# ai3DVision/CP_PFDR_graph_d1

Measured on AMD Instinct MI355X. Metric: PFDR iter/s and Medge-updates/s, 10M-vertex 6-NN graph, 1/2/4/8 MI355X, higher is better.
Workload: dtype f32; 1 GPU; PFDR_graph_quadratic_d1_l1<float>, identity A, l1 + TV, jittered 250x200x200 grid, 6-NN (V=10000000, E=60000000); global_graph=250x200x200, V_per_gpu=10000000, E_per_gpu=60000000, parallelism=single, device_inputs=True, device_bytes=3010452620, relabelled=False, split_incidence_blocks=0, tiled_blocks=39063, record_blocks=39063, slot_patterns=0, sequential_evolution=False, speculation=none, finite=True

## Files before the change

### cp_pfdr_graph_d1_amd/csrc/pfdr_quadratic.hip

```cpp
#include <cstring>
#include <stdexcept>

#include "pfdr_loop.hpp"
#include "pfdr_order.hpp"
#include "pfdr_quadratic_kernels.hpp"
#include "pfdr_sort.hpp"
#include "pfdr_sparse.hpp"
#include "pfdr_sparse_view.hpp"

namespace pfdr {

template <typename T>
static void permute(DevBuf<T> &d, const int *map, size_t n, hipStream_t s) {
    if (!d.p || !n) return;
    DevBuf<T> t(n);
    k_gather<T><<<grid_for(n), kBlock, 0, s>>>((long)n, d.p, map, t.p);
    PFDR_HIP(hipGetLastError());
    std::swap(d.p, t.p);
    std::swap(d.n, t.n);
}

__global__ void k_edge_order_keys(long E, const int *__restrict__ Eu, const int *__restrict__ where,
                                  unsigned long long *__restrict__ keys, unsigned *__restrict__ vals) {
    const long e = (long)blockIdx.x * blockDim.x + threadIdx.x;
// ... 1328 lines not shown
}

template <typename real>
void QuadSession<real>::edge_sweep(long ebeg, long eend, const Ctrl<real> *c, const char *name,
                                   long ebeg2, long eend2, const FuseDecide<real> *fd) {
    constexpr int EPT = Vec<real>::kPer16B;
    if (eend <= ebeg) { ebeg = ebeg2; eend = eend2; ebeg2 = eend2 = 0; }
    if (eend <= ebeg) return;
    hipStream_t s = stream;
    ProfScope ps(prof, name, s);
    ERange rg{ebeg, eend, ebeg2, eend2, grid_for(eend - ebeg, EPT)};
    const int nb = rg.nb0 + (eend2 > ebeg2 ? grid_for(eend2 - ebeg2, EPT) : 0);
    const int xm = xcd_fit(nb, xcd_e_), g = xcd_grid(nb, xm);
    const FuseDecide<real> f = fd ? *fd : FuseDecide<real>{};
    if (ends_ && fuse_) {
        k_edge_sweep_ends<real><<<g, kBlock, 0, s>>>(E_, xpe_.p, gie_.p, Z2_.p, A1_.p, cw_,
                                                     la_it(), la0_, rho_, c, nb, xm, f, pad_out());
        return;
    }
    constexpr long EB = kBlock * EPT;
    if (tiled_ && !fuse_ && rg.nb0 == nb && ebeg % EB == 0 && (eend % EB == 0 || eend == E_)) {
        auto k = rr_.p ? k_edge_sweep_tl<real, true, true>
                 : (!la_it() && !A1_.p) ? k_edge_sweep_tl<real, true>
                                        : k_edge_sweep_tl<real, false>;
        k<<<g, kBlock, 0, s>>>(E_, V_, Eu_.p, luv_.p, erec_.p, Ev_.p, xr_, Z2_.p, A1_.p, cw_,
                               gi_.p, la_it(), la0_, zdirect() ? nullptr : wz_.p, rho_, c,
                               (int)(ebeg / EB), nb, xm, rr_.p);
        return;
    }
    if (tiled_) throw std::logic_error("tiled edge sweep: range not on edge blocks");
    if (us_ && uptr_.p) {
        auto k = fuse_ ? k_edge_sweep_us<real, true> : k_edge_sweep_us<real, false>;
        k<<<g, kBlock, 0, s>>>(E_, Eu_.p, Ev_.p, uptr_.p, xr_, Z2_.p, A1_.p, cw_, gi_.p,
                               la_it(), la0_, wz_.p, rho_, c, nb, xm, rg, f, pad_out());
    } else {
        auto k = fuse_ ? k_edge_sweep<real, true> : k_edge_sweep<real, false>;
        k<<<g, kBlock, 0, s>>>(E_, Eu_.p, Ev_.p, xr_, Z2_.p, A1_.p, cw_, gi_.p, la_it(), la0_,
                               wz_.p, rho_, c, nb, xm, rg, f, pad_out());
    }
}

template <typename real>
void QuadSession<real>::tiny_chunk(int n) {
    const bool gated = track_ || rec_obj_;
    TinyArgs<real> t{};
    t.E = E_; t.Eu = Eu_.p; t.Ev = Ev_.p; t.Z2 = Z2_.p; t.A1 = A1_.p; t.La_d1 = la_it();
    t.la0 = la0_; t.cw = cw_; t.rho = rho_; t.gi = gi_.p; t.wz = wz_.p;
    t.va = vargs(0, nbv_, nullptr);
    t.red = red_.p; t.ctrl = gated ? ctrl_.p : nullptr; t.Dif = rec_dif_ ? Dif_.p : nullptr;
    t.track = track_ ? 1 : 0; t.iters = n;
    ProfScope ps(prof, "tiny_iterate", stream);
    k_tiny_iterate<real><<<1, kTiny, 0, stream>>>(t);
    PFDR_HIP(hipGetLastError());
}

template <typename real>
VArgs<real> QuadSession<real>::vargs(int bbeg, int bend, const Ctrl<real> *c) {
    VArgs<real> a{};
    a.V = V_; a.ptr = inc_.ptr.p; a.idx = inc_.idx.p; a.xp = xr_; a.wz = wz_.p;
    a.xpo = xw_ == xr_ ? nullptr : xw_;
    a.uptr = uptr_.p; a.mask = mask_.p; a.oidx = oidx_.p; a.blkok = blkok_.p;
    a.Y = Y_.p; a.A = A_.p; a.Ga = Ga_.p; a.Th_l1 = Th_l1_.p;
    a.prox = prox_; a.positivity = positivity_; a.lo = lo_; a.hi = hi_;
    a.fwd = mode_ == A_IDENT ? 1 : (mode_ == A_DIAG ? 2 : 0);
    a.track = track_ ? 1 : 0; a.part = vpart_.p; a.ctrl = c;
    a.late = fuse_ ? 1 : 0;
    a.E = E_;
    if (tiled_) {
        a.slots = slots_.p; a.trec = trec_.p; a.ptab = ptab_.p; a.prec = prec_.p; a.deg8 = deg8_.p; a.ustart = ustart_.p; a.tptr = tptr_.p; a.tstart = tstart_.p;
        a.tlen = tlen_.p; a.tok = tok_.p;
        a.zs = Z2_.p; a.invAux = invAux_.p; a.a0 = cw_ * la0_;
        a.gi = gi_.p;
    }
    a.l1uni = l1_uniform_ ? 1 : 0;
    a.l1u = l1u_;
    a.terms = seqdif_ ? terms_.p : nullptr;
    a.tmap = seqdif_ && reordered_ ? order_.p : nullptr;
    a.tstride = tstride_;
    a.bbeg = bbeg; a.nb = bend - bbeg; a.xcd = xcd_fit(a.nb, xcd_v_);
    a.bsplit = a.nb; a.bjump = 0;
    return a;
}

template <typename real>
void QuadSession<real>::vertex_sweep(int bbeg, int bend, const Ctrl<real> *c, const char *name,
                                     int bbeg2, int bend2) {
    if (bend <= bbeg) { bbeg = bbeg2; bend = bend2; bbeg2 = bend2 = 0; }
    if (bend <= bbeg) return;
    hipStream_t s = stream;
    VArgs<real> a = vargs(bbeg, bend, c);
    if (bend2 > bbeg2) {
        a.bsplit = bend - bbeg;
        a.bjump = bbeg2 - bend;
        a.nb += bend2 - bbeg2;
        a.xcd = xcd_fit(a.nb, xcd_v_);
    }
    ProfScope ps(prof, name, s);
    if (pad_ && bend2 <= bbeg2) {
        k_vertex_sweep_pad<real><<<xcd_grid(a.nb, a.xcd), kBlock, 0, s>>>(
            a, wzp_.p, pad_nmax_, ends_ ? pidx_.p : nullptr, ends_ ? xpe_.p : nullptr);
        return;
    }
    if (vpair_cap_ && bend2 <= bbeg2 && a.nb >= 2) {
        const int np = a.nb / 2;
        const size_t lb = 2 * (size_t)vpair_cap_ * sizeof(real);
        if (a.nb & 1) {
            VArgs<real> a1 = a;
            a1.bbeg = a.bbeg + a.nb - 1;
            a1.nb = 1;
            a1.bsplit = 1;
            a1.xcd = 0;
            if (zdirect()) k_vertex_sweep<real, 8, true><<<1, kBlock, 0, s>>>(a1);
            else k_vertex_sweep<real, 8><<<1, kBlock, 0, s>>>(a1);
        }
        a.xcd = xcd_fit(np, xcd_v_);
        const int g = xcd_grid(np, a.xcd);
        if (zdirect()) k_vertex_sweep_pair<real, true><<<g, kBlock, lb, s>>>(a, vpair_cap_);
        else k_vertex_sweep_pair<real><<<g, kBlock, lb, s>>>(a, vpair_cap_);
        return;
    }
    if (zdirect())
        k_vertex_sweep<real, 8, true><<<xcd_grid(a.nb, a.xcd), kBlock, 0, s>>>(a);
    else
        k_vertex_sweep<real, 8><<<xcd_grid(a.nb, a.xcd), kBlock, 0, s>>>(a);
}

template <typename real>
void QuadSession<real>::sweeps(const Ctrl<real> *c) {
    hipStream_t s = stream;
    if (overlap_) {
        PFDR_HIP(hipEventRecord(ev_[0], s));
        PFDR_HIP(hipStreamWaitEvent(comm_, ev_[0], 0));
        {
            ProfScope ps(prof, "halo_pull", comm_);
            halo_->pull(xr_, sizeof(R2<real>), comm_);
        }
        PFDR_HIP(hipEventRecord(ev_[1], comm_));
        edge_sweep(elo_, ehi_, c, "edge_sweep");
        PFDR_HIP(hipStreamWaitEvent(s, ev_[1], 0));
        edge_sweep(0, elo_, c, "edge_sweep_b", ehi_, E_);
        PFDR_HIP(hipEventRecord(ev_[2], s));
        PFDR_HIP(hipStreamWaitEvent(comm_, ev_[2], 0));
        {
            ProfScope ps(prof, "halo_push", comm_);
            real *src = zdirect() ? Z2_.p : wz_.p;
            halo_->push(src, src + 2 * E_, sizeof(real), comm_);
        }
        PFDR_HIP(hipEventRecord(ev_[3], comm_));
        vertex_sweep(blo_, bhi_, c, "vertex_sweep");
        PFDR_HIP(hipStreamWaitEvent(s, ev_[3], 0));
        vertex_sweep(0, blo_, c, "vertex_sweep_b", bhi_, nbv_);
    } else {
        if (halo_) {
            ProfScope ps(prof, "halo_pull", s);
            halo_->pull(xr_, sizeof(R2<real>), s);
        }
        edge_sweep(0, E_, c, "edge_sweep");
        if (halo_) {
            ProfScope ps(prof, "halo_push", s);
            real *src = zdirect() ? Z2_.p : wz_.p;
            halo_->push(src, src + 2 * E_, sizeof(real), s);
        }
        vertex_sweep(0, nbv_, c, "vertex_sweep");
    }
}

template <typename real>
void QuadSession<real>::spec_sweeps(int t, int b) {
    xr_ = xpb(t - 1);
    xw_ = xpb(t);
    real *const keep = terms_.p, *const keepp = vpart_.p;
    terms_.p += (long)b * 2 * tstride_;
    vpart_.p += (long)b * 2 * nbv_;
    sweeps(ctrl_.p);
    terms_.p = keep;
    vpart_.p = keepp;
    xr_ = xw_ = xp_.p;
}

template <typename real>
void QuadSession<real>::spec_decide(int b, hipStream_t s) {
    seq_evolution(terms_.p + (long)b * 2 * tstride_, vpart_.p + (long)b * 2 * nbv_, s);
    k_decide<real><<<1, 64, 0, s>>>(ctrl_.p, red_.p, rec_dif_ ? Dif_.p : nullptr, 1);
}

template <typename real>
void QuadSession<real>::body(int i, int n) {
    hipStream_t s = stream;
    const bool gated = track_ || rec_obj_;
    const Ctrl<real> *c = gated ? ctrl_.p : nullptr;
    if (fuse_) {
        Ctrl<real> *cb[2] = {ctrl_.p, ctrl2_.p};
        FuseDecide<real> fd{};
        if (i > 0) {
            fd.src = cb[(i - 1) & 1]; fd.dst = cb[i & 1]; fd.part = vpart_.p;
            fd.red = red_.p; fd.Dif = rec_dif_ ? Dif_.p : nullptr; fd.nparts = nbv_;
        }
        edge_sweep(0, E_, cb[0], "edge_sweep", 0, 0, &fd);
        vertex_sweep(0, nbv_, cb[i & 1], "vertex_sweep");
        if (i == n - 1) {
            FuseDecide<real> fl{cb[i & 1], cb[0], vpart_.p, red_.p, rec_dif_ ? Dif_.p : nullptr,
                                nbv_};
            k_decide_fused<real><<<1, kBlock, 0, s>>>(fl);
        }
        PFDR_HIP(hipGetLastError());
        return;
    }
// ... 308 lines not shown
```

### cp_pfdr_graph_d1_amd/csrc/pfdr_quadratic_kernels.hpp

```cpp
#pragma once
#include <algorithm>
#include <cmath>
#include <cstring>
#include <memory>
#include <type_traits>

#include "pfdr_graph.hpp"
#include "pfdr_monosum.hpp"
#include "pfdr_session.hpp"

namespace pfdr {

enum AMode : int { A_IDENT = 0, A_DIAG = 1, A_DIRECT = 2, A_ATA = 3 };
enum Prox : int { PROX_NONE = 0, PROX_L1 = 1, PROX_POS = 2, PROX_BOX = 3,
                  PROX_LO = 4, PROX_HI = 5 };
enum Gate : int { GATE_NONE = 0, GATE_ACTIVE = 1, GATE_OBJ = 2,
                  GATE_ACTIVE_OR_OBJ = 3 };

template <typename real> using R2 = typename Vec<real>::v2;

template <typename T, int N>
__device__ __forceinline__ Pk<T, N> ldv(const T *p) {
    return *reinterpret_cast<const Pk<T, N> *>(p);
}
// ... 183 lines not shown
            acc += __shfl(ng, kWave - 1, kWave);
        }
    }
    {
        const long fu = us / G;
        const int ngu = nu > 0 ? (int)((us + nu - 1) / G - fu + 1) : 0;
        for (int b = 0; b < ngu; b += kBlock * GG) {
            Slots12 d[GG];
            Pk<real, VE> x[GG][ZV];
#pragma unroll
            for (int u = 0; u < GG; u++) {
                const long g = fu + min(b + u * kBlock + tid, ngu - 1);
                d[u] = slots[g];
#pragma unroll
                for (int z = 0; z < ZV; z++) x[u][z] = ldv<real, VE>(wz + g * G + z * VE);
            }
#pragma unroll
            for (int u = 0; u < GG; u++) {
                const int k = b + u * kBlock + tid;
                if (k < ngu) {
                    const long base = (fu + k) * G;
#pragma unroll
                    for (int q = 0; q < G; q++)
                        if (base + q >= us && base + q < (long)us + nu)
                            lds[slot12(d[u], q)] = x[u][q / VE].v[q % VE];
                }
            }
        }
    }
    __syncthreads();
    const int ngv = nt ? rp[nt - 1] : 0;
    int lo = 0, end = nt ? rp[0] : 0, beg = 0;
    for (int b = 0; b < ngv; b += kBlock * GG) {
        Slots12 d[GG];
        Pk<real, VE> x[GG][ZV];
        long base[GG], A[GG];
        int L[GG];
#pragma unroll
        for (int u = 0; u < GG; u++) {
            const int k = min(b + u * kBlock + tid, ngv - 1);
            while (end <= k) {
                beg = end;
                end = rp[++lo];
            }
            A[u] = E + rs[lo];
            L[u] = rl[lo];
            base[u] = (A[u] / G + (k - beg)) * G;
        }
#pragma unroll
        for (int u = 0; u < GG; u++) {
            d[u] = slots[base[u] / G];
#pragma unroll
            for (int z = 0; z < ZV; z++) x[u][z] = ldv<real, VE>(wz + base[u] + z * VE);
        }
#pragma unroll
        for (int u = 0; u < GG; u++)
            if (b + u * kBlock + tid < ngv) {
#pragma unroll
                for (int q = 0; q < G; q++)
                    if (base[u] + q >= A[u] && base[u] + q < A[u] + L[u])
                        lds[slot12(d[u], q)] = x[u][q / VE].v[q % VE];
            }
    }
    __syncthreads();
    int my0 = dinc - dg;
    for (int q = 0; q < w; q++) my0 += wt[q];
    const int my1 = my0 + dg;
    real s = real(0);
    int j = my0;
    for (; j + 4 <= my1; j += 4) {
        const real a0 = lds[j], a1 = lds[j + 1], a2 = lds[j + 2], a3 = lds[j + 3];
        s += ZD ? wv * a0 : a0;
        s += ZD ? wv * a1 : a1;
        s += ZD ? wv * a2 : a2;
        s += ZD ? wv * a3 : a3;
    }
    for (; j < my1; j++) s += ZD ? wv * lds[j] : lds[j];
    return s;
}

constexpr int kRecRuns = 14, kTileRec = 32;
constexpr int kPrec = 16;

template <typename real, bool ZD = false>
__device__ __forceinline__ real tile_sum_rec(int V, long E, int blk, int v,
                                             const unsigned char *__restrict__ deg8,
                                             const Slots12 *__restrict__ slots,
                                             const int *__restrict__ trec,
                                             const real *__restrict__ wz, real *lds, int *wt,
                                             real wv = real(1),
                                             const Slots12 *__restrict__ ptab = nullptr,
                                             const int *__restrict__ prec = nullptr,
                                             bool pre = false, int pre_rv = 0, int pre_pr = 0,
                                             int pre_dg = 0) {
    constexpr int VE = Vec<real>::kPer16B, G = kSlotGroup, ZV = G / VE;
    const int tid = threadIdx.x, lane = tid & (kWave - 1), w = tid / kWave;
    const int dg = pre ? pre_dg : v < V ? deg8[v] : 0;
    const int rv = pre ? pre_rv : lane < kTileRec ? trec[(long)blk * kTileRec + lane] : 0;
    const int pr = pre ? pre_pr : prec && lane < kPrec ? prec[(long)blk * kPrec + lane] : 0;
    int dinc = dg;
#pragma unroll
    for (int o = 1; o < kWave; o <<= 1) {
        const int y = __shfl_up(dinc, o, kWave);
        if (lane >= o) dinc += y;
    }
    if (lane == kWave - 1) wt[w] = dinc;
    const int us = __builtin_amdgcn_readlane(rv, 0), nu = __builtin_amdgcn_readlane(rv, 1);
    const int nt = __builtin_amdgcn_readlane(rv, 2);
    const int st = __shfl(rv, min(3 + 2 * lane, kWave - 1), kWave);
    const int ln = __shfl(rv, min(4 + 2 * lane, kWave - 1), kWave);
    int P = 0;
    if (lane < nt && ln > 0) {
        const long A = E + st;
        P = (int)((A + ln - 1) / G - A / G + 1);
    }
#pragma unroll
    for (int o = 1; o < kWave; o <<= 1) {
        const int y = __shfl_up(P, o, kWave);
        if (lane >= o) P += y;
    }
    const int ngv = __builtin_amdgcn_readlane(P, kWave - 1);
    const long fu = us / G;
    const int ngu = nu > 0 ? (int)((us + nu - 1) / G - fu + 1) : 0;
    const int tot = ngu + ngv;
    for (int b = 0; b < tot; b += 2 * kBlock) {
        Slots12 d[2];
        Pk<real, VE> x[2][ZV];
        long gb[2], lo[2], hi[2];
        int pg[2];
#pragma unroll
        for (int u = 0; u < 2; u++) {
            const int k = min(b + u * kBlock + tid, tot - 1);
            const int kv = k - ngu;
            int r = 0;
            for (int q = 0; q < nt; q++) r += __builtin_amdgcn_readlane(P, q) <= kv;
            r = min(r, kWave - 1);
            const int sr = __shfl(st, r, kWave), lr = __shfl(ln, r, kWave);
            const int pb = __shfl(P, max(r - 1, 0), kWave);
            const int pv = __shfl(pr, min(r + 1, kWave - 1), kWave);
            if (k < ngu) {
                gb[u] = fu + k;
                lo[u] = us;
                hi[u] = (long)us + nu;
                pg[u] = __builtin_amdgcn_readlane(pr, 0) + k;
            } else {
                const long A = E + sr;
                const int gi = kv - (r > 0 ? pb : 0);
                gb[u] = A / G + gi;
                lo[u] = A;
                hi[u] = A + lr;
                pg[u] = pv + gi;
            }
        }
#pragma unroll
        for (int u = 0; u < 2; u++) {
            d[u] = prec ? ptab[pg[u]] : slots[gb[u]];
#pragma unroll
            for (int z = 0; z < ZV; z++) x[u][z] = ldv<real, VE>(wz + gb[u] * G + z * VE);
        }
#pragma unroll
        for (int u = 0; u < 2; u++)
            if (b + u * kBlock + tid < tot) {
#pragma unroll
                for (int q = 0; q < G; q++) {
                    const long p = gb[u] * G + q;
                    if (p >= lo[u] && p < hi[u]) lds[slot12(d[u], q)] = x[u][q / VE].v[q % VE];
                }
            }
    }
    __syncthreads();
    int my0 = dinc - dg;
    for (int q = 0; q < w; q++) my0 += wt[q];
    const int my1 = my0 + dg;
    real s = real(0);
    int j = my0;
    for (; j + 4 <= my1; j += 4) {
        const real a0 = lds[j], a1 = lds[j + 1], a2 = lds[j + 2], a3 = lds[j + 3];
        s += ZD ? wv * a0 : a0;
        s += ZD ? wv * a1 : a1;
        s += ZD ? wv * a2 : a2;
        s += ZD ? wv * a3 : a3;
    }
    for (; j < my1; j++) s += ZD ? wv * lds[j] : lds[j];
    return s;
}

template <typename real, bool ZD = false>
__device__ __forceinline__ void tile_sum_rec2(int V, long E, int b0, int v0, int v1,
                                              const unsigned char *__restrict__ deg8,
                                              const Slots12 *__restrict__ slots,
                                              const int *__restrict__ trec,
                                              const real *__restrict__ wz, real *lds, int cap,
                                              int *wt, real wv0, real wv1,
                                              const Slots12 *__restrict__ ptab,
                                              const int *__restrict__ prec, real &x0, real &x1) {
    static_assert(kTileRec == 32 && kWave == 64 && kPrec == 16, "two records per wave register");
    constexpr int VE = Vec<real>::kPer16B, G = kSlotGroup, ZV = G / VE, NW = kBlock / kWave;
    const int tid = threadIdx.x, lane = tid & (kWave - 1), w = tid / kWave;
    const int dg0 = v0 < V ? deg8[v0] : 0, dg1 = v1 < V ? deg8[v1] : 0;
    const int rv = trec[(long)b0 * kTileRec + lane];
    const int pr = prec ? prec[(long)b0 * kPrec + (lane & 31)] : 0;
    int i0 = dg0, i1 = dg1;
#pragma unroll
    for (int o = 1; o < kWave; o <<= 1) {
        const int y0 = __shfl_up(i0, o, kWave), y1 = __shfl_up(i1, o, kWave);
        if (lane >= o) {
            i0 += y0;
            i1 += y1;
        }
    }
    if (lane == kWave - 1) {
        wt[w] = i0;
        wt[NW + w] = i1;
    }
    const int us0 = __builtin_amdgcn_readlane(rv, 0), nu0 = __builtin_amdgcn_readlane(rv, 1);
    const int nt0 = __builtin_amdgcn_readlane(rv, 2);
    const int us1 = __builtin_amdgcn_readlane(rv, 32), nu1 = __builtin_amdgcn_readlane(rv, 33);
    const int nt1 = __builtin_amdgcn_readlane(rv, 34);
    const int hf = lane >> 5, rl = lane & 31;
    const int st = __shfl(rv, 32 * hf + min(3 + 2 * rl, 31), kWave);
    const int ln = __shfl(rv, 32 * hf + min(4 + 2 * rl, 31), kWave);
    int P = 0;
    if (rl < (hf ? nt1 : nt0) && ln > 0) {
        const long A = E + st;
        P = (int)((A + ln - 1) / G - A / G + 1);
    }
#pragma unroll
    for (int o = 1; o < 32; o <<= 1) {
        const int y = __shfl_up(P, o, kWave);
        if (rl >= o) P += y;
    }
    const int ngv0 = __builtin_amdgcn_readlane(P, 31), ngv1 = __builtin_amdgcn_readlane(P, 63);
    const long fu0 = us0 / G, fu1 = us1 / G;
    const int ngu0 = nu0 > 0 ? (int)((us0 + nu0 - 1) / G - fu0 + 1) : 0;
    const int ngu1 = nu1 > 0 ? (int)((us1 + nu1 - 1) / G - fu1 + 1) : 0;
    const int tot0 = ngu0 + ngv0, tot = tot0 + ngu1 + ngv1;
    const int pu0 = __builtin_amdgcn_readlane(pr, 0), pu1 = __builtin_amdgcn_readlane(pr, 16);
    for (int b = 0; b < tot; b += 2 * kBlock) {
        Slots12 d[2];
        Pk<real, VE> x[2][ZV];
        long gb[2];
        int pg[2], mt[2];
#pragma unroll
        for (int u = 0; u < 2; u++) {
            const int k = min(b + u * kBlock + tid, tot - 1);
            const int h = k >= tot0;
            const int kk = k - (h ? tot0 : 0);
            const int ngu = h ? ngu1 : ngu0;
            const int kv = kk - ngu;
            int ra = 0, rb = 0;
            for (int q = 0; q < nt0; q++) ra += __builtin_amdgcn_readlane(P, q) <= kv;
            for (int q = 0; q < nt1; q++) rb += __builtin_amdgcn_readlane(P, 32 + q) <= kv;
            const int r = min(h ? rb : ra, 31), base = 32 * h;
            const int sr = __shfl(st, base + r, kWave), lr = __shfl(ln, base + r, kWave);
            const int pb = __shfl(P, base + max(r - 1, 0), kWave);
            const int pv = __shfl(pr, 16 * h + min(r + 1, 15), kWave);
            long L, H;
            if (kk < ngu) {
                gb[u] = (h ? fu1 : fu0) + kk;
                L = h ? us1 : us0;
                H = L + (h ? nu1 : nu0);
                pg[u] = (h ? pu1 : pu0) + kk;
            } else {
                const long A = E + sr;
                const int gi = kv - (r > 0 ? pb : 0);
                gb[u] = A / G + gi;
                L = A;
                H = A + lr;
                pg[u] = pv + gi;
            }
            const int lo = (int)max(L - gb[u] * G, -1L), hi = (int)min(H - gb[u] * G, (long)G + 1);
            mt[u] = (lo + 1) | (hi + 1) << 4 | h << 8;
        }
#pragma unroll
        for (int u = 0; u < 2; u++) {
            d[u] = prec ? ptab[pg[u]] : slots[gb[u]];
#pragma unroll
            for (int z = 0; z < ZV; z++) x[u][z] = ldv<real, VE>(wz + gb[u] * G + z * VE);
        }
#pragma unroll
        for (int u = 0; u < 2; u++)
            if (b + u * kBlock + tid < tot) {
                real *l = lds + ((mt[u] >> 8) ? cap : 0);
                const int lo = (mt[u] & 15) - 1, hi = ((mt[u] >> 4) & 15) - 1;
#pragma unroll
                for (int q = 0; q < G; q++)
                    if (q >= lo && q < hi) l[slot12(d[u], q)] = x[u][q / VE].v[q % VE];
            }
    }
    __syncthreads();
    int my0 = i0 - dg0, my1 = i1 - dg1;
    for (int q = 0; q < w; q++) {
        my0 += wt[q];
        my1 += wt[NW + q];
    }
    real s0 = real(0), s1 = real(0);
    for (int j = 0; j < dg0; j++) s0 += ZD ? wv0 * lds[my0 + j] : lds[my0 + j];
    for (int j = 0; j < dg1; j++) s1 += ZD ? wv1 * lds[cap + my1 + j] : lds[cap + my1 + j];
    x0 = s0;
    x1 = s1;
}

static __global__ void k_tile_keys(long E, const int *__restrict__ Eu, const int *__restrict__ Ev,
                                   int vbits, unsigned long long *__restrict__ keys,
                                   unsigned *__restrict__ vals, int V = 0, bool split = false) {
    const long e = (long)blockIdx.x * blockDim.x + threadIdx.x;
    if (e >= E) return;
    const int u = Eu[e], v = Ev[e];
    const unsigned long long g = split && (u >= V || v >= V) ? 1ull << (2 * vbits) : 0ull;
    keys[e] = g | ((unsigned long long)(u / kBlock) << vbits) | (unsigned)(v / kBlock);
    vals[e] = (unsigned)e;
}

static __global__ void k_count_below(long n, const unsigned long long *__restrict__ keys,
                                     unsigned long long bound, unsigned long long *out) {
    long lo = 0, hi = n;
    while (lo < hi) {
        const long mid = (lo + hi) >> 1;
        if (keys[mid] < bound) lo = mid + 1;
        else hi = mid;
    }
    *out = (unsigned long long)lo;
}

static __global__ void k_tile_slots(int V, const int *__restrict__ ptr,
                                    const unsigned *__restrict__ idx,
                                    unsigned short *__restrict__ d2) {
    const int v = blockIdx.x * blockDim.x + threadIdx.x;
    if (v >= V) return;
    const int base = ptr[v - v % kBlock];
    for (int j = ptr[v]; j < ptr[v + 1]; j++) d2[idx[j]] = (unsigned short)(j - base);
}

static __global__ void k_pack_slots(long ngroups, long n, const unsigned short *__restrict__ d2,
                                    Slots12 *__restrict__ out) {
    const long g = (long)blockIdx.x * blockDim.x + threadIdx.x;
    if (g >= ngroups) return;
    unsigned long long lo = 0, hi = 0;
#pragma unroll
    for (int q = 0; q < kSlotGroup; q++) {
        const long p = g * kSlotGroup + q;
        const unsigned long long x = p < n ? (d2[p] & 0xfffu) : 0u;
        const int bit = 12 * q;
        if (bit + 12 <= 64) {
            lo |= x << bit;
        } else if (bit >= 64) {
            hi |= x << (bit - 64);
        } else {
            lo |= x << bit;
            hi |= x >> (64 - bit);
        }
    }
    Slots12 r;
    r.w[0] = (unsigned)lo;
    r.w[1] = (unsigned)(lo >> 32);
    r.w[2] = (unsigned)hi;
    out[g] = r;
}

static __global__ void k_tile_ustart(long E, int nb, const int *__restrict__ Eu,
                                     int *__restrict__ ustart) {
    const long p = (long)blockIdx.x * blockDim.x + threadIdx.x;
    if (p > E) return;
    const int lo = p == 0 ? 0 : Eu[p - 1] / kBlock + 1;
    const int hi = p == E ? nb : Eu[p] / kBlock;
    for (int b = lo; b <= hi; b++) ustart[b] = (int)p;
}

__device__ __forceinline__ int run_block(long i, const int *__restrict__ a,
                                         const unsigned long long *__restrict__ keys, int V) {
    const int x = keys ? (int)(keys[i] >> 32) : a[i];
    return x < V ? x / kBlock : -1;
}
// ... 1362 lines not shown
#pragma unroll
            for (int j = 0; j < EPT; j++) a.v[j] = cw * la.v[j];
        }
        Pk<real, EPT> ou, ov;
#pragma unroll
        for (int j = 0; j < EPT; j++)
            edge_full<real>(pu[j], pv[j], gu[j], gv[j], a.v[j], la.v[j], z.v[2 * j],
                            z.v[2 * j + 1], ou.v[j], ov.v[j], rho);
        stv<real, 2 * EPT>(Z2 + 2 * e0, z);
        if (pd.sl) {
#pragma unroll
            for (int j = 0; j < EPT; j++) {
                pd.wzp[sv.v[2 * j]] = ou.v[j];
                pd.wzp[sv.v[2 * j + 1]] = ov.v[j];
            }
        } else {
            stv<real, EPT>(wz + e0, ou);
            stv<real, EPT>(wz + E + e0, ov);
        }
    } else {
        for (long e = e0; e < eend; e++) {
            const int u = Eu[e], v = Ev[e];
            real zu = Z2[2 * e], zv = Z2[2 * e + 1], ou, ov;
            const real l = la_at(e, La_d1, la0);
            edge_full<real>(xp[u], xp[v], gi[u], gi[v], A1 ? A1[e] : cw * l, l, zu, zv, ou, ov,
                            rho);
            Z2[2 * e] = zu;
            Z2[2 * e + 1] = zv;
            if (pd.sl) {
                pd.wzp[pd.sl[2 * e]] = ou;
                pd.wzp[pd.sl[2 * e + 1]] = ov;
            } else {
                wz[e] = ou;
                wz[E + e] = ov;
            }
        }
    }
}

template <typename real>
struct VArgs {
    int V;
    int nb, xcd;
    int bbeg;
    int bsplit, bjump;
    const int *ptr;
    const unsigned *idx;
    const int *uptr;
    const unsigned *mask, *oidx;
    const int *blkok;
    const real *wz;
    R2<real> *xp;
    R2<real> *xpo;
    const real *Y, *A, *Ga, *Th_l1;
    int prox, positivity;
    real lo, hi;
    int fwd;
    int track;
    real *part;
    const Ctrl<real> *ctrl;
    int late;
    long E;
    const Slots12 *slots;
    const int *trec;
    const Slots12 *ptab;
    const int *prec;
    const unsigned char *deg8;
    const int *ustart, *tptr, *tstart, *tlen, *tok;
    const real *zs;
    const real *invAux;
    real a0;
    const R2<real> *gi;
    int l1uni;
    real l1u;
    real *terms;
    const int *tmap;
    long tstride;
};

template <typename real> struct VSweep;
template <> struct VSweep<float> { static constexpr int waves = 8; };
template <> struct VSweep<double> { static constexpr int waves = 4; };

template <typename real>
struct VOps {
    R2<real> q{};
    real th = real(0), yv = real(0), gv = real(0), av = real(0), ia = real(0);
};
template <typename real>
__device__ __forceinline__ VOps<real> vertex_ops(const VArgs<real> &a, int v,
                                                 const R2<real> *gpre = nullptr) {
    VOps<real> o;
    if (v < a.V) {
        if (a.track || !a.fwd) o.q = a.xp[v];
        real g = real(0);
        if (a.gi) {
            const R2<real> p = gpre ? *gpre : a.gi[v];
            g = p.x;
            o.ia = p.y;
        } else if (a.fwd || a.l1uni) {
            g = a.Ga[v];
        }
        if (a.prox == PROX_L1) o.th = a.l1uni ? g * a.l1u : a.Th_l1[v];
        if (a.fwd) { o.yv = a.Y[v]; o.gv = g; }
        if (a.fwd == 2) o.av = a.A[v];
    }
    return o;
}

template <typename real>
__device__ __forceinline__ R2<real> vertex_finish(const VArgs<real> &a, int v, real x,
                                                  const VOps<real> &o, real &num, real &den) {
    num = real(0);
    den = real(0);
    R2<real> q = o.q;
    const real th = o.th, yv = o.yv, gv = o.gv, av = o.av;
    if (v < a.V) {
        switch (a.prox) {
            case PROX_L1: {
                if (x > th) x -= th;
                else if (!a.positivity && (x < -th)) x += th;
                else x = real(0);
            } break;
            case PROX_POS:
                if (x < real(0)) x = real(0);
                break;
            case PROX_BOX:
                if (x < a.lo) x = a.lo;
                else if (x > a.hi) x = a.hi;
                break;
            case PROX_LO:
                if (x < a.lo) x = a.lo;
                break;
            case PROX_HI:
                if (x > a.hi) x = a.hi;
                break;
            default:
                break;
        }
        if (a.track) {
            const real d = q.x - x;
            num = d * d;
            den = x * x;
            if (a.terms) {
                const long i = a.tmap ? a.tmap[v] : v;
                a.terms[i] = num;
                a.terms[a.tstride + i] = den;
            }
        }
        q.x = x;
        if (a.fwd) {
            real p = (a.fwd == 2) ? av * x : x;
            p -= yv;
            q.y = real(2) * x - gv * p;
        }
        (a.xpo ? a.xpo : a.xp)[v] = q;
    }
    return q;
}

template <typename real, int GB, bool ZD = false>
__device__ __forceinline__ void vertex_block(const VArgs<real> &a, int blk, real *lds,
                                             real (*red)[kBlock / kWave], int *scan,
                                             int halt = 0) {
    const int v0 = blk * kBlock;
    const int v = v0 + threadIdx.x;
    const VOps<real> o = vertex_ops(a, v);
    const real wv = ZD && v < a.V ? a.a0 * (a.gi ? o.ia : a.invAux[v]) : real(1);
    real x;
    const bool pre = a.slots && a.trec;
    int pre_rv = 0, pre_pr = 0, pre_dg = 0;
    if (pre) {
        const int lane = threadIdx.x & (kWave - 1);
        pre_rv = lane < kTileRec ? a.trec[(long)blk * kTileRec + lane] : 0;
        pre_pr = a.prec && lane < kPrec ? a.prec[(long)blk * kPrec + lane] : 0;
        pre_dg = v < a.V ? a.deg8[v] : 0;
    }
    const int tk = a.slots ? a.tok[blk] : 0;
    if (tk == 2)
        x = tile_sum_rec<real, ZD>(a.V, a.E, blk, v, a.deg8, a.slots, a.trec, ZD ? a.zs : a.wz,
                                   lds, scan + 3 * kTileRuns, wv, a.ptab, a.prec, pre, pre_rv,
                                   pre_pr, pre_dg);
    else if (tk)
        x = tile_sum<real, GB, ZD>(a.V, a.E, blk, v, a.deg8, a.slots, a.ustart, a.tptr, a.tstart,
                                   a.tlen, ZD ? a.zs : a.wz, lds, scan, wv);
    else if (!ZD && a.blkok && a.blkok[blk])
        x = split_sum<real, GB>(a.V, v0, v, a.ptr, a.uptr, a.mask, a.oidx, a.wz, lds, scan);
    else
        x = gather_sum<real, GatherCap<real>::v, GB, ZD>(a.V, v0, a.ptr, a.idx,
                                                         ZD ? a.zs : a.wz, lds, wv);
    if (halt) return;
    real num, den;
    vertex_finish(a, v, x, o, num, den);
    if (a.track) {
        num = block_sum(num, red[0]);
        den = block_sum(den, red[1]);
        if (threadIdx.x == 0) {
            a.part[2 * blk] = num;
            a.part[2 * blk + 1] = den;
        }
    }
}

template <typename real, int GB, bool ZD = false>
__global__ __launch_bounds__(256, VSweep<real>::waves) void k_vertex_sweep(VArgs<real> a) {
    int halt = 0;
    if (a.ctrl) {
        if (!a.late) {
            if (a.ctrl->halt) return;
        } else {
            halt = a.ctrl->halt;
        }
    }
    __shared__ real lds[GatherCap<real>::v];
    __shared__ real red[2][kBlock / kWave];
    __shared__ int scan[3 * kTileRuns + kBlock / kWave];
    int lb = xcd_block(blockIdx.x, a.nb, a.xcd);
    if (lb >= a.nb) return;
    lb = a.nb - 1 - lb;
    if (lb >= a.bsplit) lb += a.bjump;
    vertex_block<real, GB, ZD>(a, a.bbeg + lb, lds, red, scan, halt);
}

template <typename real, bool ZD = false>
__global__ __launch_bounds__(256, 7) void k_vertex_sweep_pair(VArgs<real> a, int cap) {
    int halt = 0;
    if (a.ctrl) {
        if (!a.late) {
            if (a.ctrl->halt) return;
        } else {
            halt = a.ctrl->halt;
        }
    }
    extern __shared__ __attribute__((aligned(16))) unsigned char vpair_lds[];
    real *lds = reinterpret_cast<real *>(vpair_lds);
    __shared__ real red[2][kBlock / kWave];
    __shared__ int scan[3 * kTileRuns + 2 * (kBlock / kWave)];
    const int np = a.nb / 2;
    int lp = xcd_block(blockIdx.x, np, a.xcd);
    if (lp >= np) return;
    lp = np - 1 - lp;
    const int b0 = a.bbeg + 2 * lp;
    const int v0 = b0 * kBlock + threadIdx.x, v1 = v0 + kBlock;
    const VOps<real> o0 = vertex_ops(a, v0);
    const real wv0 = ZD && v0 < a.V ? a.a0 * (a.gi ? o0.ia : a.invAux[v0]) : real(1);
    real x0, x1;
    R2<real> g1{};
    if (a.gi && v1 < a.V) g1 = a.gi[v1];
    const real wv1 = ZD && v1 < a.V ? a.a0 * (a.gi ? g1.y : a.invAux[v1]) : real(1);
    tile_sum_rec2<real, ZD>(a.V, a.E, b0, v0, v1, a.deg8, a.slots, a.trec, ZD ? a.zs : a.wz, lds,
                            cap, scan + 3 * kTileRuns, wv0, wv1, a.ptab, a.prec, x0, x1);
    if (halt) return;
    const VOps<real> o1 = vertex_ops(a, v1, a.gi ? &g1 : nullptr);
    real n0, d0, n1, d1;
    vertex_finish(a, v0, x0, o0, n0, d0);
    vertex_finish(a, v1, x1, o1, n1, d1);
    if (a.track) {
        n0 = block_sum(n0, red[0]);
        d0 = block_sum(d0, red[1]);
        n1 = block_sum(n1, red[0]);
        d1 = block_sum(d1, red[1]);
        if (threadIdx.x == 0) {
            a.part[2 * b0] = n0;
            a.part[2 * b0 + 1] = d0;
            a.part[2 * b0 + 2] = n1;
            a.part[2 * b0 + 3] = d1;
        }
    }
}

static __global__ void k_rec_entries(int V, int nb, const int *__restrict__ ptr,
                                     const int *__restrict__ tok, int *__restrict__ out) {
    const int b = blockIdx.x * blockDim.x + threadIdx.x;
    if (b >= nb) return;
    out[b] = tok[b] == 2 ? ptr[min((b + 1) * kBlock, V)] - ptr[b * kBlock] : 0;
}

constexpr int kPadPer = 16;
template <typename real>
__global__ __launch_bounds__(256) void k_vertex_sweep_pad(VArgs<real> a,
                                                          const real *__restrict__ wzp, int nmax,
                                                          const int *__restrict__ pidx,
                                                          R2<real> *__restrict__ xpe) {
    static_assert(kPadPer * kBlock <= GatherCap<real>::v, "staged list fits the LDS chunk");
    int halt = 0;
    if (a.ctrl) {
        if (!a.late) {
            if (a.ctrl->halt) return;
        } else {
            halt = a.ctrl->halt;
        }
    }
    __shared__ real lds[kPadPer * kBlock];
    __shared__ int sidx[kPadPer * kBlock];
    __shared__ real red[2][kBlock / kWave];
    const int lb = xcd_block(blockIdx.x, a.nb, a.xcd);
    if (lb >= a.nb) return;
    const int blk = a.bbeg + lb;
    const int tid = threadIdx.x, v0 = blk * kBlock, v = v0 + tid;
    const VOps<real> o = vertex_ops(a, v);
    const int p0 = a.ptr[v0];
    const int my0 = v < a.V ? a.ptr[v] : 0, my1 = v < a.V ? a.ptr[v + 1] : 0;
    const real *src = wzp + (long)blk * nmax;
    const int per = nmax / kBlock;
    real w[kPadPer];
    int pe[kPadPer];
#pragma unroll
    for (int k = 0; k < kPadPer; k++)
        if (k < per) {
            w[k] = src[k * kBlock + tid];
            if (xpe) pe[k] = pidx[(long)blk * nmax + k * kBlock + tid];
        }
#pragma unroll
    for (int k = 0; k < kPadPer; k++)
        if (k < per) {
            lds[k * kBlock + tid] = w[k];
            if (xpe) sidx[k * kBlock + tid] = pe[k];
        }
    __syncthreads();
    real x = real(0);
    for (int j = my0; j < my1; j++) x += lds[j - p0];
    if (halt) return;
    real num, den;
    const R2<real> q = vertex_finish(a, v, x, o, num, den);
    if (xpe && v < a.V)
        for (int j = my0; j < my1; j++) xpe[sidx[j - p0]] = q;
    if (a.track) {
        num = block_sum(num, red[0]);
        den = block_sum(den, red[1]);
        if (tid == 0) {
            a.part[2 * blk] = num;
            a.part[2 * blk + 1] = den;
        }
    }
}

template <typename real>
__global__ __launch_bounds__(256) void k_edge_sweep_ends(
    long E, const R2<real> *__restrict__ xpe, const R2<real> *__restrict__ gie,
    real *__restrict__ Z2, const real *__restrict__ A1, real cw,
// ... 501 lines not shown
```

Measured before the change: 146,900 Medge-updates/s.

## Specialize vertex sweep kernels per prox mode and prefetch tile loads

Adds compile-time specialized vertex sweep and pair kernels for the identity-A, uniform-l1 or box cases, chosen on the host, so runtime flag branches and unused loads drop out. Per-vertex loads are made unconditional by clamping indices, and record/degree loads are hoisted ahead of the gather. The first batch of slot and z loads is issued before the degree prefix scan so the scan overlaps memory latency. The run-prefix scans are swapped for a 16-lane DPP row scan. The cost is more kernel instantiations and extra register pressure from holding early loads across the gather.

New measurement: 151,900 Medge-updates/s, median of 5. 1.03x the previous value.

```diff
diff --git a/cp_pfdr_graph_d1_amd/csrc/pfdr_quadratic.hip b/cp_pfdr_graph_d1_amd/csrc/pfdr_quadratic.hip
--- a/cp_pfdr_graph_d1_amd/csrc/pfdr_quadratic.hip
+++ b/cp_pfdr_graph_d1_amd/csrc/pfdr_quadratic.hip
@@ -1434,6 +1434,38 @@
     return a;
 }
 
+enum VClass : int { VC_GEN = 0, VC_L1, VC_L1_TRACK, VC_BOX };
+template <typename real>
+static VClass vclass(const VArgs<real> &a, bool zd, bool allrec) {
+    if (!zd || !allrec || !a.gi || a.fwd != 1 || !a.slots || !a.trec) return VC_GEN;
+    if (a.prox == PROX_L1 && a.l1uni) return a.track ? VC_L1_TRACK : VC_L1;
+    if (a.prox == PROX_BOX && !a.track) return VC_BOX;
+    return VC_GEN;
+}
+template <typename real>
+static auto vsweep_kernel(const VArgs<real> &a, bool zd, bool allrec)
+    -> void (*)(VArgs<real>) {
+    switch (vclass(a, zd, allrec)) {
+        case VC_L1: return k_vertex_sweep<real, 8, true, VIdent<PROX_L1, false>>;
+        case VC_L1_TRACK: return k_vertex_sweep<real, 8, true, VIdent<PROX_L1, true>>;
+        case VC_BOX: return k_vertex_sweep<real, 8, true, VIdent<PROX_BOX, false>>;
+        default: break;
+    }
+    return zd ? k_vertex_sweep<real, 8, true> : k_vertex_sweep<real, 8>;
+}
+template <typename real>
+static auto vpair_kernel(const VArgs<real> &a, bool zd) -> void (*)(VArgs<real>, int) {
+    if constexpr (sizeof(real) == 4) {
+        switch (vclass(a, zd, true)) {
+            case VC_L1: return k_vertex_sweep_pair<real, true, VIdent<PROX_L1, false>>;
+            case VC_L1_TRACK: return k_vertex_sweep_pair<real, true, VIdent<PROX_L1, true>>;
+            case VC_BOX: return k_vertex_sweep_pair<real, true, VIdent<PROX_BOX, false>>;
+            default: break;
+        }
+    }
+    return zd ? k_vertex_sweep_pair<real, true> : k_vertex_sweep_pair<real>;
+}
+
 template <typename real>
 void QuadSession<real>::vertex_sweep(int bbeg, int bend, const Ctrl<real> *c, const char *name,
                                      int bbeg2, int bend2) {
@@ -1462,19 +1494,15 @@
             a1.nb = 1;
             a1.bsplit = 1;
             a1.xcd = 0;
-            if (zdirect()) k_vertex_sweep<real, 8, true><<<1, kBlock, 0, s>>>(a1);
-            else k_vertex_sweep<real, 8><<<1, kBlock, 0, s>>>(a1);
+            vsweep_kernel(a1, zdirect(), true)<<<1, kBlock, 0, s>>>(a1);
         }
         a.xcd = xcd_fit(np, xcd_v_);
         const int g = xcd_grid(np, a.xcd);
-        if (zdirect()) k_vertex_sweep_pair<real, true><<<g, kBlock, lb, s>>>(a, vpair_cap_);
-        else k_vertex_sweep_pair<real><<<g, kBlock, lb, s>>>(a, vpair_cap_);
+        vpair_kernel(a, zdirect())<<<g, kBlock, lb, s>>>(a, vpair_cap_);
         return;
     }
-    if (zdirect())
-        k_vertex_sweep<real, 8, true><<<xcd_grid(a.nb, a.xcd), kBlock, 0, s>>>(a);
-    else
-        k_vertex_sweep<real, 8><<<xcd_grid(a.nb, a.xcd), kBlock, 0, s>>>(a);
+    const bool allrec = tiled_ && record_blocks == grid_for(V_);
+    vsweep_kernel(a, zdirect(), allrec)<<<xcd_grid(a.nb, a.xcd), kBlock, 0, s>>>(a);
 }
 
 template <typename real>
diff --git a/cp_pfdr_graph_d1_amd/csrc/pfdr_quadratic_kernels.hpp b/cp_pfdr_graph_d1_amd/csrc/pfdr_quadratic_kernels.hpp
--- a/cp_pfdr_graph_d1_amd/csrc/pfdr_quadratic_kernels.hpp
+++ b/cp_pfdr_graph_d1_amd/csrc/pfdr_quadratic_kernels.hpp
@@ -289,29 +289,28 @@
 constexpr int kRecRuns = 14, kTileRec = 32;
 constexpr int kPrec = 16;
 
+template <typename T>
+__device__ __forceinline__ void keep_below(T &x) {
+    asm volatile("" : "+v"(x));
+}
+
+__device__ __forceinline__ int row_incl_scan(int x) {
+    x += __builtin_amdgcn_update_dpp(0, x, 0x111, 0xf, 0xf, false);
+    x += __builtin_amdgcn_update_dpp(0, x, 0x112, 0xf, 0xf, false);
+    x += __builtin_amdgcn_update_dpp(0, x, 0x114, 0xf, 0xf, false);
+    x += __builtin_amdgcn_update_dpp(0, x, 0x118, 0xf, 0xf, false);
+    return x;
+}
+
 template <typename real, bool ZD = false>
-__device__ __forceinline__ real tile_sum_rec(int V, long E, int blk, int v,
-                                             const unsigned char *__restrict__ deg8,
+__device__ __forceinline__ real tile_sum_rec(int V, long E, int v, int rv, int pr, int dg,
                                              const Slots12 *__restrict__ slots,
-                                             const int *__restrict__ trec,
                                              const real *__restrict__ wz, real *lds, int *wt,
-                                             real wv = real(1),
-                                             const Slots12 *__restrict__ ptab = nullptr,
-                                             const int *__restrict__ prec = nullptr,
-                                             bool pre = false, int pre_rv = 0, int pre_pr = 0,
-                                             int pre_dg = 0) {
+                                             real a0, real ia,
+                                             const Slots12 *__restrict__ ptab, bool pat) {
+    static_assert(kRecRuns <= 16, "the runs' prefix is a scan over one row of 16 lanes");
     constexpr int VE = Vec<real>::kPer16B, G = kSlotGroup, ZV = G / VE;
     const int tid = threadIdx.x, lane = tid & (kWave - 1), w = tid / kWave;
-    const int dg = pre ? pre_dg : v < V ? deg8[v] : 0;
-    const int rv = pre ? pre_rv : lane < kTileRec ? trec[(long)blk * kTileRec + lane] : 0;
-    const int pr = pre ? pre_pr : prec && lane < kPrec ? prec[(long)blk * kPrec + lane] : 0;
-    int dinc = dg;
-#pragma unroll
-    for (int o = 1; o < kWave; o <<= 1) {
-        const int y = __shfl_up(dinc, o, kWave);
-        if (lane >= o) dinc += y;
-    }
-    if (lane == kWave - 1) wt[w] = dinc;
     const int us = __builtin_amdgcn_readlane(rv, 0), nu = __builtin_amdgcn_readlane(rv, 1);
     const int nt = __builtin_amdgcn_readlane(rv, 2);
     const int st = __shfl(rv, min(3 + 2 * lane, kWave - 1), kWave);
@@ -321,19 +320,15 @@
         const long A = E + st;
         P = (int)((A + ln - 1) / G - A / G + 1);
     }
-#pragma unroll
-    for (int o = 1; o < kWave; o <<= 1) {
-        const int y = __shfl_up(P, o, kWave);
-        if (lane >= o) P += y;
-    }
-    const int ngv = __builtin_amdgcn_readlane(P, kWave - 1);
+    P = row_incl_scan(P);
+    const int ngv = __builtin_amdgcn_readlane(P, 15);
     const long fu = us / G;
     const int ngu = nu > 0 ? (int)((us + nu - 1) / G - fu + 1) : 0;
     const int tot = ngu + ngv;
-    for (int b = 0; b < tot; b += 2 * kBlock) {
-        Slots12 d[2];
-        Pk<real, VE> x[2][ZV];
-        long gb[2], lo[2], hi[2];
+    Slots12 d[2];
+    Pk<real, VE> x[2][ZV];
+    long gb[2], lo[2], hi[2];
+    const auto issue = [&](int b) __attribute__((always_inline)) {
         int pg[2];
 #pragma unroll
         for (int u = 0; u < 2; u++) {
@@ -361,10 +356,12 @@
         }
 #pragma unroll
         for (int u = 0; u < 2; u++) {
-            d[u] = prec ? ptab[pg[u]] : slots[gb[u]];
+            d[u] = pat ? ptab[pg[u]] : slots[gb[u]];
 #pragma unroll
             for (int z = 0; z < ZV; z++) x[u][z] = ldv<real, VE>(wz + gb[u] * G + z * VE);
         }
+    };
+    const auto stage = [&](int b) __attribute__((always_inline)) {
 #pragma unroll
         for (int u = 0; u < 2; u++)
             if (b + u * kBlock + tid < tot) {
@@ -374,16 +371,31 @@
                     if (p >= lo[u] && p < hi[u]) lds[slot12(d[u], q)] = x[u][q / VE].v[q % VE];
                 }
             }
+    };
+    if (tot > 0) issue(0);
+    int dinc = dg;
+#pragma unroll
+    for (int o = 1; o < kWave; o <<= 1) {
+        const int y = __shfl_up(dinc, o, kWave);
+        if (lane >= o) dinc += y;
+    }
+    if (lane == kWave - 1) wt[w] = dinc;
+    if (tot > 0) stage(0);
+    for (int b = 2 * kBlock; b < tot; b += 2 * kBlock) {
+        issue(b);
+        stage(b);
     }
     __syncthreads();
+    keep_below(ia);
+    const real wv = ZD && v < V ? a0 * ia : real(1);
     int my0 = dinc - dg;
     for (int q = 0; q < w; q++) my0 += wt[q];
     const int my1 = my0 + dg;
     real s = real(0);
     int j = my0;
     for (; j + 4 <= my1; j += 4) {
-        const real a0 = lds[j], a1 = lds[j + 1], a2 = lds[j + 2], a3 = lds[j + 3];
-        s += ZD ? wv * a0 : a0;
+        const real a0_ = lds[j], a1 = lds[j + 1], a2 = lds[j + 2], a3 = lds[j + 3];
+        s += ZD ? wv * a0_ : a0_;
         s += ZD ? wv * a1 : a1;
         s += ZD ? wv * a2 : a2;
         s += ZD ? wv * a3 : a3;
@@ -393,33 +405,17 @@
 }
 
 template <typename real, bool ZD = false>
-__device__ __forceinline__ void tile_sum_rec2(int V, long E, int b0, int v0, int v1,
-                                              const unsigned char *__restrict__ deg8,
+__device__ __forceinline__ void tile_sum_rec2(int V, long E, int v0, int v1, int rv, int pr,
+                                              int dg0, int dg1,
                                               const Slots12 *__restrict__ slots,
-                                              const int *__restrict__ trec,
                                               const real *__restrict__ wz, real *lds, int cap,
-                                              int *wt, real wv0, real wv1,
-                                              const Slots12 *__restrict__ ptab,
-                                              const int *__restrict__ prec, real &x0, real &x1) {
+                                              int *wt, real a0, real ia0, real ia1,
+                                              const Slots12 *__restrict__ ptab, bool pat,
+                                              real &x0, real &x1) {
     static_assert(kTileRec == 32 && kWave == 64 && kPrec == 16, "two records per wave register");
+    static_assert(kRecRuns <= 16, "each block's prefix is a scan over one row of 16 lanes");
     constexpr int VE = Vec<real>::kPer16B, G = kSlotGroup, ZV = G / VE, NW = kBlock / kWave;
     const int tid = threadIdx.x, lane = tid & (kWave - 1), w = tid / kWave;
-    const int dg0 = v0 < V ? deg8[v0] : 0, dg1 = v1 < V ? deg8[v1] : 0;
-    const int rv = trec[(long)b0 * kTileRec + lane];
-    const int pr = prec ? prec[(long)b0 * kPrec + (lane & 31)] : 0;
-    int i0 = dg0, i1 = dg1;
-#pragma unroll
-    for (int o = 1; o < kWave; o <<= 1) {
-        const int y0 = __shfl_up(i0, o, kWave), y1 = __shfl_up(i1, o, kWave);
-        if (lane >= o) {
-            i0 += y0;
-            i1 += y1;
-        }
-    }
-    if (lane == kWave - 1) {
-        wt[w] = i0;
-        wt[NW + w] = i1;
-    }
     const int us0 = __builtin_amdgcn_readlane(rv, 0), nu0 = __builtin_amdgcn_readlane(rv, 1);
     const int nt0 = __builtin_amdgcn_readlane(rv, 2);
     const int us1 = __builtin_amdgcn_readlane(rv, 32), nu1 = __builtin_amdgcn_readlane(rv, 33);
@@ -432,22 +428,19 @@
         const long A = E + st;
         P = (int)((A + ln - 1) / G - A / G + 1);
     }
-#pragma unroll
-    for (int o = 1; o < 32; o <<= 1) {
-        const int y = __shfl_up(P, o, kWave);
-        if (rl >= o) P += y;
-    }
-    const int ngv0 = __builtin_amdgcn_readlane(P, 31), ngv1 = __builtin_amdgcn_readlane(P, 63);
+    P = row_incl_scan(P);
+    const int ngv0 = __builtin_amdgcn_readlane(P, 15), ngv1 = __builtin_amdgcn_readlane(P, 47);
     const long fu0 = us0 / G, fu1 = us1 / G;
     const int ngu0 = nu0 > 0 ? (int)((us0 + nu0 - 1) / G - fu0 + 1) : 0;
     const int ngu1 = nu1 > 0 ? (int)((us1 + nu1 - 1) / G - fu1 + 1) : 0;
     const int tot0 = ngu0 + ngv0, tot = tot0 + ngu1 + ngv1;
     const int pu0 = __builtin_amdgcn_readlane(pr, 0), pu1 = __builtin_amdgcn_readlane(pr, 16);
-    for (int b = 0; b < tot; b += 2 * kBlock) {
-        Slots12 d[2];
-        Pk<real, VE> x[2][ZV];
+    Slots12 d[2];
+    Pk<real, VE> x[2][ZV];
+    int mt[2];
+    const auto issue = [&](int b) __attribute__((always_inline)) {
         long gb[2];
-        int pg[2], mt[2];
+        int pg[2];
 #pragma unroll
         for (int u = 0; u < 2; u++) {
             const int k = min(b + u * kBlock + tid, tot - 1);
@@ -481,10 +474,12 @@
         }
 #pragma unroll
         for (int u = 0; u < 2; u++) {
-            d[u] = prec ? ptab[pg[u]] : slots[gb[u]];
+            d[u] = pat ? ptab[pg[u]] : slots[gb[u]];
 #pragma unroll
             for (int z = 0; z < ZV; z++) x[u][z] = ldv<real, VE>(wz + gb[u] * G + z * VE);
         }
+    };
+    const auto stage = [&](int b) __attribute__((always_inline)) {
 #pragma unroll
         for (int u = 0; u < 2; u++)
             if (b + u * kBlock + tid < tot) {
@@ -494,8 +489,31 @@
                 for (int q = 0; q < G; q++)
                     if (q >= lo && q < hi) l[slot12(d[u], q)] = x[u][q / VE].v[q % VE];
             }
+    };
+    if (tot > 0) issue(0);
+    int i0 = dg0, i1 = dg1;
+#pragma unroll
+    for (int o = 1; o < kWave; o <<= 1) {
+        const int y0 = __shfl_up(i0, o, kWave), y1 = __shfl_up(i1, o, kWave);
+        if (lane >= o) {
+            i0 += y0;
+            i1 += y1;
+        }
+    }
+    if (lane == kWave - 1) {
+        wt[w] = i0;
+        wt[NW + w] = i1;
+    }
+    if (tot > 0) stage(0);
+    for (int b = 2 * kBlock; b < tot; b += 2 * kBlock) {
+        issue(b);
+        stage(b);
     }
     __syncthreads();
+    keep_below(ia0);
+    keep_below(ia1);
+    const real wv0 = ZD && v0 < V ? a0 * ia0 : real(1);
+    const real wv1 = ZD && v1 < V ? a0 * ia1 : real(1);
     int my0 = i0 - dg0, my1 = i1 - dg1;
     for (int q = 0; q < w; q++) {
         my0 += wt[q];
@@ -2024,33 +2042,69 @@
 template <> struct VSweep<float> { static constexpr int waves = 8; };
 template <> struct VSweep<double> { static constexpr int waves = 4; };
 
+#define PFDR_VSW template <typename real> static __device__ __forceinline__
+struct VGen {
+    static constexpr bool gen = true;
+    PFDR_VSW bool gi(const VArgs<real> &a) { return a.gi != nullptr; }
+    PFDR_VSW bool l1uni(const VArgs<real> &a) { return a.l1uni != 0; }
+    PFDR_VSW int fwd(const VArgs<real> &a) { return a.fwd; }
+    PFDR_VSW bool track(const VArgs<real> &a) { return a.track != 0; }
+    PFDR_VSW int prox(const VArgs<real> &a) { return a.prox; }
+};
+template <int PROX, bool TRACK>
+struct VIdent {
+    static constexpr bool gen = false;
+    PFDR_VSW bool gi(const VArgs<real> &) { return true; }
+    PFDR_VSW bool l1uni(const VArgs<real> &) { return true; }
+    PFDR_VSW int fwd(const VArgs<real> &) { return 1; }
+    PFDR_VSW bool track(const VArgs<real> &) { return TRACK; }
+    PFDR_VSW int prox(const VArgs<real> &) { return PROX; }
+};
+#undef PFDR_VSW
+
 template <typename real>
 struct VOps {
     R2<real> q{};
     real th = real(0), yv = real(0), gv = real(0), av = real(0), ia = real(0);
 };
-template <typename real>
-__device__ __forceinline__ VOps<real> vertex_ops(const VArgs<real> &a, int v,
-                                                 const R2<real> *gpre = nullptr) {
+template <typename real, class S = VGen, bool ZD = false>
+__device__ __forceinline__ void vertex_load_w(const VArgs<real> &a, int vc, VOps<real> &o) {
+    if (S::gi(a)) {
+        const R2<real> p = a.gi[vc];
+        o.gv = p.x;
+        o.ia = p.y;
+    } else if (ZD) {
+        o.ia = a.invAux[vc];
+    }
+}
+template <typename real, class S = VGen>
+__device__ __forceinline__ void vertex_load_rest(const VArgs<real> &a, int vc, VOps<real> &o) {
+    if (S::track(a) || !S::fwd(a)) o.q = a.xp[vc];
+    if (!S::gi(a) && (S::fwd(a) || S::l1uni(a))) o.gv = a.Ga[vc];
+    if (S::prox(a) == PROX_L1 && !S::l1uni(a)) o.th = a.Th_l1[vc];
+    if (S::fwd(a)) o.yv = a.Y[vc];
+    if (S::fwd(a) == 2) o.av = a.A[vc];
+}
+template <typename real, class S = VGen, bool ZD = false>
+__device__ __forceinline__ VOps<real> vertex_loads(const VArgs<real> &a, int v) {
     VOps<real> o;
-    if (v < a.V) {
-        if (a.track || !a.fwd) o.q = a.xp[v];
-        real g = real(0);
-        if (a.gi) {
-            const R2<real> p = gpre ? *gpre : a.gi[v];
-            g = p.x;
-            o.ia = p.y;
-        } else if (a.fwd || a.l1uni) {
-            g = a.Ga[v];
-        }
-        if (a.prox == PROX_L1) o.th = a.l1uni ? g * a.l1u : a.Th_l1[v];
-        if (a.fwd) { o.yv = a.Y[v]; o.gv = g; }
-        if (a.fwd == 2) o.av = a.A[v];
-    }
+    const int vc = min(v, a.V - 1);
+    vertex_load_w<real, S, ZD>(a, vc, o);
+    vertex_load_rest<real, S>(a, vc, o);
     return o;
 }
-
-template <typename real>
+template <typename real, class S = VGen>
+__device__ __forceinline__ void vertex_derive(const VArgs<real> &a, VOps<real> &o) {
+    if (S::prox(a) == PROX_L1 && S::l1uni(a)) o.th = o.gv * a.l1u;
+}
+template <typename real>
+__device__ __forceinline__ VOps<real> vertex_ops(const VArgs<real> &a, int v) {
+    VOps<real> o = vertex_loads(a, v);
+    vertex_derive(a, o);
+    return o;
+}
+
+template <typename real, class S = VGen>
 __device__ __forceinline__ R2<real> vertex_finish(const VArgs<real> &a, int v, real x,
                                                   const VOps<real> &o, real &num, real &den) {
     num = real(0);
@@ -2058,7 +2112,7 @@
     R2<real> q = o.q;
     const real th = o.th, yv = o.yv, gv = o.gv, av = o.av;
     if (v < a.V) {
-        switch (a.prox) {
+        switch (S::prox(a)) {
             case PROX_L1: {
                 if (x > th) x -= th;
                 else if (!a.positivity && (x < -th)) x += th;
@@ -2080,7 +2134,7 @@
             default:
                 break;
         }
-        if (a.track) {
+        if (S::track(a)) {
             const real d = q.x - x;
             num = d * d;
             den = x * x;
@@ -2091,8 +2145,8 @@
             }
         }
         q.x = x;
-        if (a.fwd) {
-            real p = (a.fwd == 2) ? av * x : x;
+        if (S::fwd(a)) {
+            real p = (S::fwd(a) == 2) ? av * x : x;
             p -= yv;
             q.y = real(2) * x - gv * p;
         }
@@ -2101,40 +2155,48 @@
     return q;
 }
 
-template <typename real, int GB, bool ZD = false>
+template <typename real, int GB, bool ZD = false, class S = VGen>
 __device__ __forceinline__ void vertex_block(const VArgs<real> &a, int blk, real *lds,
                                              real (*red)[kBlock / kWave], int *scan,
                                              int halt = 0) {
     const int v0 = blk * kBlock;
     const int v = v0 + threadIdx.x;
-    const VOps<real> o = vertex_ops(a, v);
-    const real wv = ZD && v < a.V ? a.a0 * (a.gi ? o.ia : a.invAux[v]) : real(1);
-    real x;
-    const bool pre = a.slots && a.trec;
-    int pre_rv = 0, pre_pr = 0, pre_dg = 0;
+    const bool tiled = !S::gen || a.slots;
+    const bool pre = !S::gen || (a.slots && a.trec);
+    int rv = 0, pr = 0, dg = 0;
     if (pre) {
         const int lane = threadIdx.x & (kWave - 1);
-        pre_rv = lane < kTileRec ? a.trec[(long)blk * kTileRec + lane] : 0;
-        pre_pr = a.prec && lane < kPrec ? a.prec[(long)blk * kPrec + lane] : 0;
-        pre_dg = v < a.V ? a.deg8[v] : 0;
-    }
-    const int tk = a.slots ? a.tok[blk] : 0;
-    if (tk == 2)
-        x = tile_sum_rec<real, ZD>(a.V, a.E, blk, v, a.deg8, a.slots, a.trec, ZD ? a.zs : a.wz,
-                                   lds, scan + 3 * kTileRuns, wv, a.ptab, a.prec, pre, pre_rv,
-                                   pre_pr, pre_dg);
-    else if (tk)
-        x = tile_sum<real, GB, ZD>(a.V, a.E, blk, v, a.deg8, a.slots, a.ustart, a.tptr, a.tstart,
-                                   a.tlen, ZD ? a.zs : a.wz, lds, scan, wv);
-    else if (!ZD && a.blkok && a.blkok[blk])
-        x = split_sum<real, GB>(a.V, v0, v, a.ptr, a.uptr, a.mask, a.oidx, a.wz, lds, scan);
-    else
-        x = gather_sum<real, GatherCap<real>::v, GB, ZD>(a.V, v0, a.ptr, a.idx,
-                                                         ZD ? a.zs : a.wz, lds, wv);
+        const int *pp = a.prec ? a.prec + (long)blk * kPrec : a.trec + (long)blk * kTileRec;
+        pr = pp[lane & (kPrec - 1)];
+        rv = a.trec[(long)blk * kTileRec + (lane & (kTileRec - 1))];
+        if (lane >= kTileRec) rv = 0;
+        dg = a.deg8[min(v, a.V - 1)];
+        if (v >= a.V) dg = 0;
+    }
+    VOps<real> o = vertex_loads<real, S, ZD>(a, v);
+    const int tk = !S::gen ? 2 : tiled ? a.tok[blk] : 0;
+    real x;
+    if (tk == 2) {
+        x = tile_sum_rec<real, ZD>(a.V, a.E, v, rv, pr, dg, a.slots, ZD ? a.zs : a.wz, lds,
+                                   scan + 3 * kTileRuns, a.a0, o.ia, a.ptab, a.prec != nullptr);
+    } else {
+        real ia = o.ia;
+        keep_below(ia);
+        const real wv = ZD && v < a.V ? a.a0 * ia : real(1);
+        if (tk)
+            x = tile_sum<real, GB, ZD>(a.V, a.E, blk, v, a.deg8, a.slots, a.ustart, a.tptr,
+                                       a.tstart, a.tlen, ZD ? a.zs : a.wz, lds, scan, wv);
+        else if (!ZD && a.blkok && a.blkok[blk])
+            x = split_sum<real, GB>(a.V, v0, v, a.ptr, a.uptr, a.mask, a.oidx, a.wz, lds, scan);
+        else
+            x = gather_sum<real, GatherCap<real>::v, GB, ZD>(a.V, v0, a.ptr, a.idx,
+                                                             ZD ? a.zs : a.wz, lds, wv);
+    }
     if (halt) return;
+    vertex_derive<real, S>(a, o);
     real num, den;
-    vertex_finish(a, v, x, o, num, den);
-    if (a.track) {
+    vertex_finish<real, S>(a, v, x, o, num, den);
+    if (S::track(a)) {
         num = block_sum(num, red[0]);
         den = block_sum(den, red[1]);
         if (threadIdx.x == 0) {
@@ -2144,7 +2206,7 @@
     }
 }
 
-template <typename real, int GB, bool ZD = false>
+template <typename real, int GB, bool ZD = false, class S = VGen>
 __global__ __launch_bounds__(256, VSweep<real>::waves) void k_vertex_sweep(VArgs<real> a) {
     int halt = 0;
     if (a.ctrl) {
@@ -2161,10 +2223,10 @@
     if (lb >= a.nb) return;
     lb = a.nb - 1 - lb;
     if (lb >= a.bsplit) lb += a.bjump;
-    vertex_block<real, GB, ZD>(a, a.bbeg + lb, lds, red, scan, halt);
-}
-
-template <typename real, bool ZD = false>
+    vertex_block<real, GB, ZD, S>(a, a.bbeg + lb, lds, red, scan, halt);
+}
+
+template <typename real, bool ZD = false, class S = VGen>
 __global__ __launch_bounds__(256, 7) void k_vertex_sweep_pair(VArgs<real> a, int cap) {
     int halt = 0;
     if (a.ctrl) {
@@ -2184,20 +2246,29 @@
     lp = np - 1 - lp;
     const int b0 = a.bbeg + 2 * lp;
     const int v0 = b0 * kBlock + threadIdx.x, v1 = v0 + kBlock;
-    const VOps<real> o0 = vertex_ops(a, v0);
-    const real wv0 = ZD && v0 < a.V ? a.a0 * (a.gi ? o0.ia : a.invAux[v0]) : real(1);
+    const int lane = threadIdx.x & (kWave - 1);
+    const int *pp = a.prec ? a.prec + (long)b0 * kPrec : a.trec + (long)b0 * kTileRec;
+    const int pr = pp[lane & 31];
+    const int rv = a.trec[(long)b0 * kTileRec + lane];
+    int dg0 = a.deg8[min(v0, a.V - 1)], dg1 = a.deg8[min(v1, a.V - 1)];
+    if (v0 >= a.V) dg0 = 0;
+    if (v1 >= a.V) dg1 = 0;
+    VOps<real> o0 = vertex_loads<real, S, ZD>(a, v0);
+    VOps<real> o1;
+    vertex_load_w<real, S, ZD>(a, min(v1, a.V - 1), o1);
+    if (!S::gen) vertex_load_rest<real, S>(a, min(v1, a.V - 1), o1);
     real x0, x1;
-    R2<real> g1{};
-    if (a.gi && v1 < a.V) g1 = a.gi[v1];
-    const real wv1 = ZD && v1 < a.V ? a.a0 * (a.gi ? g1.y : a.invAux[v1]) : real(1);
-    tile_sum_rec2<real, ZD>(a.V, a.E, b0, v0, v1, a.deg8, a.slots, a.trec, ZD ? a.zs : a.wz, lds,
-                            cap, scan + 3 * kTileRuns, wv0, wv1, a.ptab, a.prec, x0, x1);
+    tile_sum_rec2<real, ZD>(a.V, a.E, v0, v1, rv, pr, dg0, dg1, a.slots, ZD ? a.zs : a.wz, lds,
+                            cap, scan + 3 * kTileRuns, a.a0, o0.ia, o1.ia, a.ptab,
+                            a.prec != nullptr, x0, x1);
     if (halt) return;
-    const VOps<real> o1 = vertex_ops(a, v1, a.gi ? &g1 : nullptr);
+    if (S::gen) vertex_load_rest<real, S>(a, min(v1, a.V - 1), o1);
+    vertex_derive<real, S>(a, o0);
+    vertex_derive<real, S>(a, o1);
     real n0, d0, n1, d1;
-    vertex_finish(a, v0, x0, o0, n0, d0);
-    vertex_finish(a, v1, x1, o1, n1, d1);
-    if (a.track) {
+    vertex_finish<real, S>(a, v0, x0, o0, n0, d0);
+    vertex_finish<real, S>(a, v1, x1, o1, n1, d1);
+    if (S::track(a)) {
         n0 = block_sum(n0, red[0]);
         d0 = block_sum(d0, red[1]);
         n1 = block_sum(n1, red[0]);
```
